# casiacob/ip-parallel-optimal-control

Hardware: AMD Instinct MI355X
Metric: KKT Newton-steps/sec at (horizon N x batch) (higher is better)
Workload: dtype f64; 1 GPU; cartpole nx=4 nu=1 N=200 global batch=4096 (BASELINE c3), 4096 per GPU; layout=tiled, horizon=200, batch_per_gpu=4096, global_batch=4096, lanes_per_trajectory=32, parallelism=trajectory-sharded x1

## Files before the change

### include/noc_hip.h

```cpp
#ifndef NOC_HIP_H
#define NOC_HIP_H

#ifdef __cplusplus
extern "C" {
#endif

#define NOC_ABI_VERSION 5

int noc_abi_version(void);
const char* noc_build_hash(void);
const char* noc_last_error(void);
int noc_kkt_supported(int nx, int nu);
int noc_kkt_default_lanes(int nx, int nu, int N);
int noc_kkt_pick_lanes(int nx, int nu, int N, int B);
int noc_kkt_gains_on_chip(int nx, int nu, int N, int lanes);
void noc_debug_set_ablation(int bits);

int noc_kkt_solve(int nx, int nu, int N, int B, int lanes,
                  const double* A, const double* Bm, const double* Q, const double* R,
                  const double* M, const double* r, const double* q, const double* c,
                  const double* P, const double* p, const double* x0, const double* reg,
                  const int* active,
                  double* dx, double* du, double* pred, int* feasible,
                  double* K, double* d, double* S, double* v, void* stream);
// ... 53 lines not shown
  int Bt, N;
  int lanes;
  int flags;
  double *x, *u, *x0;
  double *A, *B, *Q, *R, *M, *r, *P;
  double *cx, *cu, *lc, *lam;
  double *dx, *du, *pred, *K, *d;
  int *feasible;
  int *phase, *kkt_active, *it, *inner, *total_it, *kkt_solves;
  int *repeats;
  const int *order;
  double *bp, *rp, *rinc, *cost, *hu, *gnorm, *reg;
} noc_ipm_ws;

int noc_family_supported(const noc_family* fam);
int noc_ipm_init(const noc_ipm_ws* ws, double bp0, void* stream);
int noc_ipm_prepare(const noc_family* fam, const noc_ipm_ws* ws, int mode, int terminal,
                    void* stream);
int noc_ipm_trial(const noc_family* fam, const noc_ipm_ws* ws, int mode, void* stream);
int noc_ipm_step(const noc_family* fam, const noc_ipm_ws* ws, int mode, int terminal, int lanes,
                 void* stream);
int noc_ipm_rollout(const noc_family* fam, const noc_ipm_ws* ws, void* stream);
int noc_ipm_step_main(const noc_family* fam, const noc_ipm_ws* ws, int mode, int terminal,
                      void* stream);
int noc_ipm_promote(const noc_ipm_ws* ws, void* stream);

#define NOC_FIELD_A 0
#define NOC_FIELD_B 1
#define NOC_FIELD_Q 2
#define NOC_FIELD_R 3
#define NOC_FIELD_M 4
int noc_kkt_compact_supported(const noc_family* fam, int N, int lanes);
int noc_compact_width(const noc_family* fam, int field);
int noc_kkt_solve_compact(const noc_family* fam, int N, int B, int lanes,
                          const double* A, const double* Bm, const double* Q, const double* R,
                          const double* M, const double* r, const double* P, const double* x0,
                          const double* reg, const int* active,
                          double* dx, double* du, double* pred, int* feasible,
                          double* K, double* d, double* S, double* v, void* stream);
int noc_blocks_expand(const noc_family* fam, int N, int B, int lanes,
                      const double* cA, const double* cB, const double* cQ, const double* cR,
                      const double* cM, double* A, double* Bm, double* Q, double* R, double* M,
                      void* stream);
int noc_ipm_prepare_compact(const noc_family* fam, const noc_ipm_ws* ws, int mode, int terminal,
                            void* stream);
int noc_ipm_step_compact(const noc_family* fam, const noc_ipm_ws* ws, int mode, int terminal,
                         int lanes, void* stream);
int noc_ipm_step_main_compact(const noc_family* fam, const noc_ipm_ws* ws, int mode, int terminal,
                              void* stream);

int noc_ipm_solve_supported(const noc_family* fam, int N, int lanes);
int noc_debug_phase_cycles(long long* out, int n, int reset);
int noc_debug_traj_times(long long* out, int n);
int noc_ipm_solve(const noc_family* fam, const noc_ipm_ws* ws, int mode, int terminal, double bp0,
                  int max_solves, void* stream);

#define NOC_TRAJ_PARAM_DOUBLES 32
#define NOC_TP_GOAL 0
#define NOC_TP_WX 8
#define NOC_TP_WU 16
#define NOC_TP_WF 20
#define NOC_TP_UBOUND 28
int noc_traj_params_supported(const noc_family* fam, int N, int lanes);
int noc_ipm_solve_params(const noc_family* fam, const noc_ipm_ws* ws, const double* params,
                         int mode, int terminal, double bp0, int max_solves, void* stream);
int noc_ipm_prepare_params(const noc_family* fam, const noc_ipm_ws* ws, const double* params,
// ... 65 lines not shown
```

### ip-parallel-optimal-control_amd/csrc/block_struct.h

```cpp
#pragma once
#include <hip/hip_runtime.h>

#include <cstdint>
#include <utility>

#include "ipm_family.h"

namespace noc {

template <class F, int... I>
NOC_DEV void static_for_seq(F&& f, std::integer_sequence<int, I...>) {
  (f(std::integral_constant<int, I>{}), ...);
}
template <int N, class F>
NOC_DEV void static_for(F&& f) {
  static_for_seq(f, std::make_integer_sequence<int, N>{});
}

enum BlockKind : int {
  BK_VAR = 0,
  BK_ZERO,
  BK_ONE,
  BK_DT,
  BK_EXPR_A,
  BK_EXPR_B,
  BK_LIT,
  BK_PA,
  BK_PB,
  BK_WX
};

template <int N>
struct KindTable {
  int kind[N] = {};
  int pos[N] = {};
  int idx[N] = {};
  double lit[N] = {};
  double delta[N] = {};
  int nv = 0;
};

template <int KIND, int NX, int NU>
struct GenPattern {
  static constexpr int NZ = NX + NU;
  static constexpr bool kLinear = KIND == NOC_FAMILY_LINEAR;
  static constexpr bool kDiscrete = Fam<KIND, NX, NU>::kDiscrete;
  static constexpr bool kGenCost = Fam<KIND, NX, NU>::kGenCost;
  static constexpr bool jvar(int k) {
    if constexpr (KIND == NOC_FAMILY_PENDULUM) return gen::pendulum_jac_var[k] != 0;
    else if constexpr (KIND == NOC_FAMILY_CARTPOLE) return gen::cartpole_jac_var[k] != 0;
// ... 114 lines not shown
  for (int i = 0; i < NU; ++i)
    for (int j = i; j < NU; ++j) {
      const int e = Sym<NU>::idx(i, j);
      const bool h = G::hnz((NX + i) * G::NZ + NX + j) || G::hnz((NX + j) * G::NZ + NX + i);
      const int ci = NX * NX + i * NU + j, cj = NX * NX + j * NU + i;
      if (!ON || h || i == j) kt_set(t, e, BK_VAR);
      else if (G::kGenCost) {
        if (G::cvar(ci) || G::cvar(cj)) kt_set(t, e, BK_VAR);
        else kt_set(t, e, BK_LIT, 0.5 * (G::cconst(ci) + G::cconst(cj)));
      } else {
        kt_set(t, e, BK_ZERO);
      }
    }
  return t;
}
template <int KIND, int NX, int NU, bool ON>
constexpr KindTable<NX * NU> table_M() {
  using G = GenPattern<KIND, NX, NU>;
  KindTable<NX * NU> t{};
  for (int i = 0; i < NX; ++i)
    for (int j = 0; j < NU; ++j) {
      const int e = i * NU + j, ck = NX * NX + NU * NU + e;
      if (!ON || G::hnz(i * G::NZ + NX + j)) kt_set(t, e, BK_VAR);
      else if (G::kGenCost) {
        if (G::cvar(ck)) kt_set(t, e, BK_VAR);
        else kt_set(t, e, BK_LIT, G::cconst(ck));
      } else {
        kt_set(t, e, BK_ZERO);
      }
    }
  return t;
}

template <int N>
constexpr uint64_t nz_mask(const KindTable<N>& t) {
  uint64_t m = 0;
  for (int e = 0; e < N; ++e)
    if (t.kind[e] != BK_ZERO) m |= (uint64_t)1 << e;
  return m;
}

template <int KIND, int NX, int NU, bool ON>
struct BlockStruct {
  static_assert(NX * NX <= 64, "structure masks hold up to 64 entries");
  static constexpr bool kOn = ON;
  template <int F>
  static constexpr auto table() {
    if constexpr (F == BF_A) return table_A<KIND, NX, NU, ON>();
    else if constexpr (F == BF_B) return table_B<KIND, NX, NU, ON>();
    else if constexpr (F == BF_Q) return table_Q<KIND, NX, NU, ON>();
    else if constexpr (F == BF_R) return table_R<KIND, NX, NU, ON>();
    else return table_M<KIND, NX, NU, ON>();
  }
  template <int F>
  static constexpr int size() {
    if constexpr (F == BF_A) return NX * NX;
    else if constexpr (F == BF_B || F == BF_M) return NX * NU;
    else if constexpr (F == BF_Q) return Sym<NX>::SZ;
    else return Sym<NU>::SZ;
  }
  template <int F>
  static constexpr int nv() { return table<F>().nv; }
  static constexpr uint64_t kNzA = nz_mask(table_A<KIND, NX, NU, ON>());
  static constexpr uint64_t kNzB = nz_mask(table_B<KIND, NX, NU, ON>());
  static constexpr bool nzA(int k, int j) { return ((kNzA >> (k * NX + j)) & 1) != 0; }
  static constexpr bool nzB(int k, int j) { return ((kNzB >> (k * NU + j)) & 1) != 0; }
// ... 58 lines not shown
```

### ip-parallel-optimal-control_amd/csrc/kkt_compact.hip

```cpp
#include <hip/hip_runtime.h>

#include "../../include/noc_hip.h"
#include "block_struct.h"
#include "noc_internal.h"
#include "small_linalg.h"

namespace noc {

#ifndef NOC_CUSTOM_FAMILY
template <int KIND, int NX, int NU, int L>
hipError_t launch_kkt_compact(const noc_family& prm, const KKTArgs& a, hipStream_t stream);

#define NOC_COMPACT_FAMILIES(X) X(NOC_FAMILY_CARTPOLE, 4, 1) X(NOC_FAMILY_PENDULUM, 2, 1)

template <int KIND, int NX, int NU>
__global__ __launch_bounds__(256) void blocks_expand_kernel(noc_family prm, ExpandArgs e) {
  using BS = BlockStruct<KIND, NX, NU, true>;
  const long long t = (long long)blockIdx.x * blockDim.x + threadIdx.x;
  const int L = e.lanes;
  const Chunks ch(e.N, L);
  if (t >= (long long)e.B * ch.cmax * L) return;
  const int b = (int)(t / ((long long)ch.cmax * L));
  const int rem = (int)(t % ((long long)ch.cmax * L));
  const int j = rem / L, l = rem % L;
// ... 25 lines not shown
    default: return -1;
  }
}

template <int KIND, int NX, int NU>
static hipError_t dispatch_t(const noc_family& p, const KKTArgs& a, int lanes, hipStream_t stream) {
  switch (lanes) {
    case 64: return launch_kkt_compact<KIND, NX, NU, 64>(p, a, stream);
    case 32: return launch_kkt_compact<KIND, NX, NU, 32>(p, a, stream);
    case 16: return launch_kkt_compact<KIND, NX, NU, 16>(p, a, stream);
    case 8: return launch_kkt_compact<KIND, NX, NU, 8>(p, a, stream);
    default: return hipErrorInvalidValue;
  }
}

static bool compact_family(const noc_family& p) {
#define X(K, NX, NU) if (p.kind == K && p.nx == NX && p.nu == NU) return true;
  NOC_COMPACT_FAMILIES(X)
#undef X
  return false;
}

bool kkt_compact_supported(const noc_family& p, int lanes) {
  return compact_family(p) && (lanes == 8 || lanes == 16 || lanes == 32 || lanes == 64);
}

int compact_width(const noc_family& p, int field) {
#define X(K, NX, NU) if (p.kind == K && p.nx == NX && p.nu == NU) return width_t<K, NX, NU>(field);
  NOC_COMPACT_FAMILIES(X)
#undef X
  return -1;
}

hipError_t kkt_compact_dispatch(const noc_family& p, const KKTArgs& a, int lanes, hipStream_t stream) {
#define X(K, NX, NU) if (p.kind == K && p.nx == NX && p.nu == NU) return dispatch_t<K, NX, NU>(p, a, lanes, stream);
  NOC_COMPACT_FAMILIES(X)
#undef X
  return hipErrorInvalidValue;
}

hipError_t blocks_expand(const noc_family& p, const ExpandArgs& e, hipStream_t stream) {
  const long long cmax = (e.N + e.lanes - 1) / e.lanes;
  const unsigned grid = (unsigned)(((long long)e.B * cmax * e.lanes + 255) / 256);
#define X(K, NX, NU)                                                                              \
  if (p.kind == K && p.nx == NX && p.nu == NU) {                                                  \
    hipLaunchKernelGGL((blocks_expand_kernel<K, NX, NU>), dim3(grid), dim3(256), 0, stream, p, e); \
    return hipGetLastError();                                                                     \
  }
  NOC_COMPACT_FAMILIES(X)
#undef X
  return hipErrorInvalidValue;
}

#else

bool kkt_compact_supported(const noc_family&, int) { return false; }
int compact_width(const noc_family&, int) { return -1; }
hipError_t kkt_compact_dispatch(const noc_family&, const KKTArgs&, int, hipStream_t) { return hipErrorInvalidValue; }
hipError_t blocks_expand(const noc_family&, const ExpandArgs&, hipStream_t) { return hipErrorInvalidValue; }

#endif

}
```

### ip-parallel-optimal-control_amd/csrc/kkt_compact_src.h

```cpp
#pragma once
#include <hip/hip_runtime.h>

#include "block_struct.h"
#include "kkt_scan_impl.h"

namespace noc {

template <class BS, int NX, int NU, int L>
struct CompactSrc {
  using Struct = BS;
  const KKTArgs& a;
  const noc_family& p;
  int traj, l, cmax;
  size_t tN;
  template <int F, bool LAST = false>
  NOC_DEV void field(const double* base, int j, double* full) const {
    constexpr int EV = BS::template nv<F>();
    double v[EV > 0 ? EV : 1];
    if constexpr (EV > 0) tload_pol<EV, L, LAST>(base, traj, j, l, cmax, v);
    BS::template expand<F>(p, v, full);
  }
  template <int PART, bool LAST = false>
  NOC_DEV void stage_part(int s, int j, double reg, StageData<NX, NU>& st) const {
    constexpr bool REST = PART != 2, WQ = PART != 1, WAB = REST && PART != 3;
    (void)s;
    (void)reg;
    if constexpr (WAB) {
      field<BF_A>(a.A, j, st.A.v);
      field<BF_B>(a.Bm, j, st.B.v);
    }
    if constexpr (WQ) field<BF_Q, LAST>(a.Q, j, st.Q.v);
    if constexpr (REST) {
      field<BF_R, LAST>(a.R, j, st.R.v);
      field<BF_M, LAST>(a.M, j, st.M.v);
      tload_pol<NU, L, LAST>(a.r, traj, j, l, cmax, st.r.v);
    }
  }
  NOC_DEV void stage(int s, int j, double reg, StageData<NX, NU>& st) const { stage_part<0>(s, j, reg, st); }
  NOC_DEV void stage_last(int s, int j, double reg, StageData<NX, NU>& st) const {
    stage_part<0, true>(s, j, reg, st);
  }
  NOC_DEV void ab(int s, int j, Mat<NX, NX>& A, Mat<NX, NU>& Bm, Vec<NX>& c) const {
    (void)s;
    field<BF_A, true>(a.A, j, A.v);
    field<BF_B, true>(a.Bm, j, Bm.v);
    set_zero(c);
  }
  NOC_DEV void cvec(int, int, Vec<NX>& c) const { set_zero(c); }
};

template <int KIND, int NX, int NU, int L, int CACHE, bool BIG>
__global__ __launch_bounds__(256, BIG ? 1 : NOC_KKT_WAVES_PER_SIMD) void kkt_scan_compact_kernel(noc_family prm,
                                                                                             KKTArgs a) {
  static_assert(L <= 64, "one-wave segments");
  const int tid = blockIdx.x * blockDim.x + threadIdx.x;
  if constexpr (BIG) asm volatile("" ::: "a255");
  const int traj = tid / L;
  const bool dead = traj >= a.B || (a.active && a.active[traj] == 0);
  const bool wave_live = __any(!dead);
  if (dead) {
    if (!wave_live && a.lds_out && a.mode != MODE_BWD && !(a.ablate & 6)) __syncthreads();
    return;
  }
  using BS = BlockStruct<KIND, NX, NU, true>;
  const int l = tid % L;
  const int cmax = a.N / L + (a.N % L ? 1 : 0);
  const CompactSrc<BS, NX, NU, L> src{a, prm, traj, l, cmax, (size_t)traj * a.N};
  kkt_scan_wave_src<NX, NU, L, false, true, CompactSrc<BS, NX, NU, L>, CACHE, true, BIG, false, false, false,
                    true>(a, traj, l, src);
}

template <int KIND, int NX, int NU, int L>
hipError_t launch_kkt_compact(const noc_family& prm, const KKTArgs& a_in, hipStream_t stream) {
  KKTArgs a = a_in;
  const long long threads = (long long)a.B * L;
  constexpr int CC = kkt_cache_len<NX, NU, L>();
  const int cmax = a.N / L + (a.N % L ? 1 : 0);
  const bool cached = CC > 0 && cmax <= CC && !(a.ablate & 8);
  constexpr bool kHasBig = (L == 64 || L == 32) && NX >= 3 && NX <= 4;
  const bool big = kHasBig && (threads + 63) / 64 <= kkt_device_simds() && kkt_big_enabled();
  const size_t slots1 = (a.mode == MODE_BWD || (!a.dx && !a.du)) ? 0 : kkt_lds_bytes_rt(NX, NU, a.N, L);
  const int wpb = kkt_waves_per_block((threads + 63) / 64, slots1);
  const size_t lds = slots1 * wpb;
  a.lds_out = slots1 > 0 ? 1 : 0;
  a.ab_slots = 0;
  a.lds_base = 0;
  a.tiled = 1;
  const int block = 64 * wpb;
  const unsigned grid = (unsigned)((threads + block - 1) / block);
  if (!a.lds_out && (!a.K || !a.d)) return hipErrorInvalidValue;
  if (cached) {
    if constexpr (CC > 0)
      hipLaunchKernelGGL((kkt_scan_compact_kernel<KIND, NX, NU, L, CC, false>), dim3(grid), dim3(block), lds, stream,
                         prm, a);
  } else if (big) {
    if constexpr (kHasBig)
      hipLaunchKernelGGL((kkt_scan_compact_kernel<KIND, NX, NU, L, 0, true>), dim3(grid), dim3(block), lds, stream,
                         prm, a);
  } else {
    hipLaunchKernelGGL((kkt_scan_compact_kernel<KIND, NX, NU, L, 0, false>), dim3(grid), dim3(block), lds, stream,
                       prm, a);
  }
  return hipGetLastError();
}

}
```

### ip-parallel-optimal-control_amd/csrc/kkt_scan_impl.h

```cpp
#pragma once
#include <hip/hip_runtime.h>

#include <type_traits>

#include "small_linalg.h"
#include "noc_internal.h"

#pragma clang fp contract(fast)

#ifndef NOC_KKT_WAVES_PER_SIMD
#define NOC_KKT_WAVES_PER_SIMD 2
#endif


namespace noc {

#ifdef NOC_SCAN_STAMPS
constexpr int kStampWaves = 65536, kStampSlots = 8;
__device__ long long g_scan_stamps[kStampWaves][kStampSlots][2];
#define NOC_STAMP(i)                                                                         \
  do {                                                                                       \
    const unsigned wv_ = (blockIdx.x * blockDim.x + threadIdx.x) >> 6;                      \
    if ((threadIdx.x & 63) == 0 && wv_ < kStampWaves) {                                      \
      g_scan_stamps[wv_][i][0] = (long long)__builtin_amdgcn_s_memrealtime();                \
// ... 449 lines not shown
    NOC_UNROLL for (int k = 0; k < NX; ++k) s += Y[k][i] * w[k];
    e1.nu[i] = s;
  }
  set_zero(e1.A);
  set_zero(e1.b);
  set_zero(e1.C);
}

template <int NX, int NU, int L, bool AFF, bool TILED>
struct ArgsSrc {
  using Struct = DenseBlocks<NX, NU>;
  const KKTArgs& a;
  int traj, l, cmax;
  size_t tN;
  NOC_DEV void stage(int s, int j, double reg, StageData<NX, NU>& st) const {
    load_stage<NX, NU, L, AFF, TILED>(a, traj, tN + s, j, l, cmax, reg, st);
  }
  template <int PART, bool LAST = false>
  NOC_DEV void stage_part(int s, int j, double reg, StageData<NX, NU>& st) const {
    load_stage<NX, NU, L, AFF, TILED, PART, LAST>(a, traj, tN + s, j, l, cmax, reg, st);
  }
  NOC_DEV void stage_last(int s, int j, double reg, StageData<NX, NU>& st) const {
    load_stage<NX, NU, L, AFF, TILED, 0, true>(a, traj, tN + s, j, l, cmax, reg, st);
  }
  NOC_DEV void ab(int s, int j, Mat<NX, NX>& A, Mat<NX, NU>& Bm, Vec<NX>& c) const {
    load_AB<NX, NU, L, AFF, TILED>(a, traj, tN + s, j, l, cmax, A, Bm, c);
  }
  NOC_DEV void cvec(int s, int j, Vec<NX>& c) const {
    if constexpr (TILED) tload<NX, L>(a.c, traj, j, l, cmax, c.v);
    else gload<NX>(a.c + (tN + s) * NX, c.v);
  }
};

template <int NX, int NU, int L, bool AFF, bool TILED, class SRC, int CACHE = 0, bool HANDOFF = true,
          bool BIG = false, bool NT3 = false, bool AB = (BIG && ab_supported<NX, NU>()), bool IO0 = false,
          bool PEEL = false>
NOC_DEV void kkt_scan_wave_src(const KKTArgs& a, const int traj, const int l, const SRC& src) {
  constexpr int KD = kd_width<NX, NU>();
  using ST = typename SRC::Struct;
  if (traj >= a.B) return;
  if (a.active && a.active[traj] == 0) return;
  const int N = a.N;
  const int base = N / L, rem = N % L;
  const int len = base + (l < rem ? 1 : 0);
  const int start = l * base + (l < rem ? l : rem);
  const bool last = (l == L - 1);
  const int io = IO0 ? 0 : traj;
  const double reg = a.reg ? a.reg[io] : 0.0;
  const size_t tN = (size_t)traj * N;
  const int cmax = base + (rem ? 1 : 0);
  constexpr int LW = L > 64 ? 64 : L;
  constexpr int W = L / LW;
  static_assert(W == 1 || W == 2, "segments of up to two waves");
  const int wv = l / LW, lw = l % LW;
  double* join = nullptr;
  if constexpr (W > 1) join = lds_join<NX, NU>(N, a.lds_out != 0);
  (void)wv;
  (void)lw;
  (void)join;
  lds_double* lab = nullptr;
  int abn = 0;
  if constexpr (AB) {
    abn = (CACHE == 0 && a.mode != MODE_FWD && !(a.ablate & (16 | 64))) ? a.ab_slots : 0;
    if (abn > 0) lab = lds_ab<NX, NU>(a.lds_base, a.ab_slots);
  }
  NOC_STAMP_DECL;
  NOC_STAMP(0);
  StageData<NX, NU> cache[CACHE > 0 ? CACHE : 1];
  if constexpr (CACHE > 0) {
    if (a.mode != MODE_FWD) {
      NOC_UNROLL for (int jj = 0; jj < CACHE; ++jj)
        if (jj < len) src.stage(start + jj, jj, reg, cache[jj]);
    }
  }

  Mat<NX, NX> Phi;
  Vec<NX> phi;
  Mat<NX, NX> hA;
  Mat<NX, NU> hB;
  Vec<NX> hc;
  bool handed = false;
  SRC src_re = src;
  if (a.ablate & 16) { src_re.traj = traj & 1; src_re.tN = (size_t)(traj & 1) * N; }
  if (a.mode != MODE_FWD) {
    Elem<NX> e;
    set_zero(e.b);
    set_zero(e.C);
    if (last) {
      set_zero(e.A);
      set_zero(e.nu);
      gload_sym<NX, true>(a.P + (size_t)traj * NX * NX, e.J);
      if constexpr (AFF) { if (a.p) gload<NX>(a.p + (size_t)traj * NX, e.nu.v); }
    } else {
      set_identity(e.A);
      set_zero(e.nu);
      set_zero(e.J);
    }
    if constexpr (CACHE > 0) {
      NOC_UNROLL for (int jj = CACHE - 1; jj >= 0; --jj)
        if (jj < len) prepend<NX, NU, AFF, ST>(e, cache[jj], reg);
    } else {
      for (int s = start + len - 1; s >= start; --s) {
        StageData<NX, NU> st;
        src.stage(s, s - start, reg, st);
        if constexpr (AB) { if (s - start < abn) ab_store<NX, NU>(lab, s - start, st.A, st.B); }
        prepend<NX, NU, AFF, ST>(e, st, reg);
      }
    }
    NOC_STAMP(1); NOC_ISA_MARK("phase", 1);
    if constexpr (W == 1) {
      if (!(a.ablate & 1)) rev_scan_sklansky<NX, L, 0, (NX <= 2 || BIG)>(e);
    } else {
      if (!(a.ablate & 1)) {
        combine_sklansky<NX, false, 0, true>(e);
// ... 149 lines not shown
          NOC_UNROLL for (int j = 0; j < NX; ++j) {
            double u = 0.0;
            NOC_UNROLL for (int k = 0; k < NX; ++k) if (ST::nzF(k, j)) u += Phi(i, k) * F(k, j);
            Pn(i, j) = u;
          }
        }
        Phi = Pn;
      }
    };
    const int sfirst = start + len - 1;
    constexpr std::true_type kFirst{};
    constexpr std::false_type kLater{};
    if constexpr (CACHE > 0) {
      NOC_UNROLL for (int jj = CACHE - 1; jj >= 0; --jj)
        if (jj < len) riccati_stage(start + jj, cache[jj], jj == len - 1);
    } else {
      bool split = false;
      if constexpr (AB) split = abn > 0;
      if (split) {
        if constexpr (AB) {
          const int jl = len < abn ? len : abn;
          for (int s = start + len - 1; s >= start + jl; --s) {
            StageData<NX, NU> st;
            stage3(s, st);
            riccati_stage(s, st, s == sfirst);
          }
          for (int s = start + jl - 1; s >= start; --s) {
            StageData<NX, NU> st;
            src_re.template stage_part<3, NT3>(s, s - start, reg, st);
            ab_load<NX, NU>(lab, s - start, st.A, st.B);
            riccati_stage(s, st, s == sfirst);
          }
        }
      } else if constexpr (HANDOFF) {
        int s = sfirst;
        if (PEEL && len > 1) {
          StageData<NX, NU> st;
          stage3(s, st);
          riccati_stage(s, st, kFirst);
          --s;
        }
        for (; s > start; --s) {
          StageData<NX, NU> st;
          stage3(s, st);
          riccati_stage(s, st, kLater);
        }
        if (len > 0) {
          StageData<NX, NU> st;
          stage3(start, st);
          riccati_stage(start, st, len == 1);
          hA = st.A;
          hB = st.B;
          if constexpr (AFF) hc = st.c; else set_zero(hc);
          handed = a.mode == MODE_FULL && !(a.ablate & 32);
        }
      } else {
        for (int s = start + len - 1; s >= start; --s) {
          StageData<NX, NU> st;
          stage3(s, st);
          riccati_stage(s, st, s == sfirst);
        }
      }
    }
    segment_sum_and<LW>(pred, feas, (int)__lane_id());
    if constexpr (W > 1) {
      constexpr int PO = Sym<NX>::SZ + 2 * NX;
// ... 31 lines not shown
          NOC_UNROLL for (int u = 0; u < NU; ++u) if (ST::nzB(i, u)) t += Bm(i, u) * Kk[u * NX + j];
          F(i, j) = t;
        }
        double t = cc[i];
        NOC_UNROLL for (int u = 0; u < NU; ++u) if (ST::nzB(i, u)) t += Bm(i, u) * Kk[NU * NX + u];
        f[i] = t;
      }
      Mat<NX, NX> Pn;
      NOC_UNROLL for (int i = 0; i < NX; ++i) {
        double t = phi[i];
        NOC_UNROLL for (int k = 0; k < NX; ++k) if (AFF || ST::nzf(k)) t += Phi(i, k) * f[k];
        phi[i] = t;
        NOC_UNROLL for (int j = 0; j < NX; ++j) {
          double u = 0.0;
          NOC_UNROLL for (int k = 0; k < NX; ++k) if (ST::nzF(k, j)) u += Phi(i, k) * F(k, j);
          Pn(i, j) = u;
        }
      }
      Phi = Pn;
    }
  }

  Vec<NX> x0;
  set_zero(x0);
  if (a.x0) gload<NX>(a.x0 + (size_t)traj * NX, x0.v);
  if (l == 0) {
    NOC_UNROLL for (int i = 0; i < NX; ++i) {
      double t = phi[i];
      NOC_UNROLL for (int k = 0; k < NX; ++k) t += Phi(i, k) * x0[k];
      phi[i] = t;
    }
    set_zero(Phi);
  }
  affine_prefix_sklansky<NX, LW>(Phi, phi);
  Vec<NX> x;
  wave_shift_up1<NX>(phi.v, x.v);
  if (l == 0) x = x0;
  if constexpr (W > 1) {
    constexpr int XO = Sym<NX>::SZ + NX;
    if (wv == 0 && lw == LW - 1) NOC_UNROLL for (int i = 0; i < NX; ++i) join[XO + i] = phi[i];
    Mat<NX, NX> oP;
    if (wv == 1) wave_shift_up1<NX * NX>(Phi.v, oP.v);
    __syncthreads();
    if (wv == 1) {
      Vec<NX> xw;
      NOC_UNROLL for (int i = 0; i < NX; ++i) xw[i] = join[XO + i];
      if (lw == 0) {
        x = xw;
      } else {
        NOC_UNROLL for (int i = 0; i < NX; ++i) {
          double t = x[i];
          NOC_UNROLL for (int k = 0; k < NX; ++k) t += oP(i, k) * xw[k];
          x[i] = t;
        }
      }
    }
  }
  NOC_STAMP(4); NOC_ISA_MARK("phase", 4);
  double* slot = lds_slots<NX, NU, L>(N);
  const bool via_lds = a.lds_out != 0;
  const bool kd_lds = via_lds && a.mode == MODE_FULL;
  Mat<NX, NX> nA;
  Mat<NX, NU> nB;
  double nK[NU * (NX + 1)];
  Vec<NX> nc;
  auto fetch = [&](int s) {
// ... 40 lines not shown
            NOC_UNROLL for (int i = 0; i < NU * (NX + 1); ++i) Kk[i] = slot[s * KD + i];
          } else {
            load_Kd<NX, NU, L, TILED>(a, traj, tN + s, jj, l, cmax, Kk);
          }
          Vec<NX> cc;
          if constexpr (AFF) cc = cache[jj].c; else set_zero(cc);
          fwd_stage(s, cache[jj].A, cache[jj].B, cc, Kk);
        }
      }
    }
  } else {
    int s0 = start;
    if constexpr (AB) {
      if (abn > 0) {
        const int jl = len < abn ? len : abn;
        for (int s = start; s < start + jl; ++s) {
          Mat<NX, NX> A;
          Mat<NX, NU> Bm;
          Vec<NX> cc;
          ab_load<NX, NU>(lab, s - start, A, Bm);
          set_zero(cc);
          if constexpr (AFF) { if (a.c) src_re.cvec(s, s - start, cc); }
          double Kk[NU * (NX + 1)];
          if (kd_lds) {
            NOC_UNROLL for (int i = 0; i < NU * (NX + 1); ++i) Kk[i] = slot[s * KD + i];
          } else {
            load_Kd<NX, NU, L, TILED>(a, traj, tN + s, s - start, l, cmax, Kk);
          }
          fwd_stage(s, A, Bm, cc, Kk);
        }
        s0 = start + jl;
      }
    }
    if (s0 < start + len) {
      if (handed && s0 == start) {
        nA = hA;
        nB = hB;
        nc = hc;
        if (kd_lds) {
          NOC_UNROLL for (int i = 0; i < NU * (NX + 1); ++i) nK[i] = slot[start * KD + i];
        } else {
          load_Kd<NX, NU, L, TILED>(a, traj, tN + start, 0, l, cmax, nK);
        }
      } else {
        fetch(s0);
      }
    }
    for (int s = s0; s < start + len; ++s) {
      const Mat<NX, NX> A = nA;
      const Mat<NX, NU> Bm = nB;
      const Vec<NX> cc = nc;
      double Kk[NU * (NX + 1)];
      NOC_UNROLL for (int i = 0; i < NU * (NX + 1); ++i) Kk[i] = nK[i];
      if (s + 1 < start + len) fetch(s + 1);
      fwd_stage(s, A, Bm, cc, Kk);
    }
  }
  NOC_STAMP(5); NOC_ISA_MARK("phase", 5);
  if (!via_lds) {
    if (last && a.dx) gstore<NX>(a.dx + (tN + traj + N) * NX, x.v);
    return;
  }
  if (last) NOC_UNROLL for (int i = 0; i < NX; ++i) slot[N * KD + i] = x[i];
  __syncthreads();
  if (a.dx) {
    double* dst = a.dx + (tN + traj) * NX;
    if constexpr (NX % 2 == 0) {
      constexpr int H = NX / 2;
      double2* dst2 = reinterpret_cast<double2*>(dst);
      for (int i = l; i < (N + 1) * H; i += L) {
        const int s = i / H, e = 2 * (i - s * H);
        noc_dbl2 v;
        v.x = slot[s * KD + e];
        v.y = slot[s * KD + e + 1];
        __builtin_nontemporal_store(v, reinterpret_cast<noc_dbl2*>(dst2 + i));
      }
    } else {
      for (int i = l; i < (N + 1) * NX; i += L) {
        const int s = i / NX;
        dst[i] = slot[s * KD + (i - s * NX)];
      }
    }
  }
  if (a.du) {
    double* dst = a.du + tN * NU;
    for (int i = l; i < N * NU; i += L) {
      const int s = i / NU;
      dst[i] = slot[s * KD + NX + (i - s * NU)];
    }
  }
  NOC_STAMP(6);
}

template <int NX, int NU, int L, bool AFF, bool TILED, int CACHE = 0, bool HANDOFF = true,
          bool BIG = false, bool NT3 = false>
NOC_DEV void kkt_scan_wave(const KKTArgs& a, const int traj, const int l) {
  const int cmax = a.N / L + (a.N % L ? 1 : 0);
  const ArgsSrc<NX, NU, L, AFF, TILED> src{a, traj, l, cmax, (size_t)traj * a.N};
  kkt_scan_wave_src<NX, NU, L, AFF, TILED, ArgsSrc<NX, NU, L, AFF, TILED>, CACHE, HANDOFF, BIG, NT3,
                    (BIG && ab_supported<NX, NU>()), false, true>(a, traj, l, src);
}

template <int NX, int NU, int L, bool AFF, bool TILED, int CACHE, bool BIG = false, bool NT3 = false>
__global__ __launch_bounds__(L > 64 ? L : 256, (L > 64 || BIG) ? 1 : NOC_KKT_WAVES_PER_SIMD) void kkt_scan_kernel(KKTArgs a) {
  const int tid = blockIdx.x * blockDim.x + threadIdx.x;
  if constexpr (L > 64 || BIG) asm volatile("" ::: "a255");
  const int traj = tid / L;
  if constexpr (L <= 64) {
    const bool dead = traj >= a.B || (a.active && a.active[traj] == 0);
    const bool wave_live = __any(!dead);
    if (dead) {
      if (!wave_live && a.lds_out && a.mode != MODE_BWD && !(a.ablate & 6)) __syncthreads();
      return;
    }
  }
  kkt_scan_wave<NX, NU, L, AFF, TILED, CACHE, true, BIG, NT3 && TILED && CACHE == 0>(a, traj, tid % L);
}

template <int NX, int NU, int L>
constexpr int kkt_cache_len() { return (NX <= 2 && L >= 32) ? 2 : 0; }


template <int NX, int NU, int L, bool AFF>
hipError_t launch_kkt(const KKTArgs& a_in, hipStream_t stream) {
// ... 90 lines not shown
```

### ip-parallel-optimal-control_amd/csrc/noc_abi.hip

```cpp
#include <hip/hip_runtime.h>

#include <cstdint>
#include <cstdio>
#include <string>

#include "../../include/noc_hip.h"
#include "noc_internal.h"
#include "small_linalg.h"

namespace noc {
static std::string kkt_shapes_str();
}

namespace {
thread_local std::string g_last_error;
int g_ablate = 0;

int fail(int code, const std::string& msg) {
  g_last_error = msg;
  return code;
}

int check_ptr(const void* p, const char* name, bool required, unsigned align = 16) {
  if (!p) return required ? fail(-2, std::string("required pointer is NULL: ") + name) : 0;
// ... 144 lines not shown
                    "kkt_scan launch");
}

int noc_kkt_solve(int nx, int nu, int N, int B, int lanes, const double* A, const double* Bm,
                  const double* Q, const double* R, const double* M, const double* r,
                  const double* q, const double* c, const double* P, const double* p,
                  const double* x0, const double* reg, const int* active, double* dx, double* du,
                  double* pred, int* feasible, double* K, double* d, double* S, double* v,
                  void* stream) {
  return kkt_common(noc::MODE_FULL, 0, nx, nu, N, B, lanes, A, Bm, Q, R, M, r, q, c, P, p, x0, reg,
                    active, dx, du, pred, feasible, K, d, S, v, stream);
}

int noc_kkt_solve_tiled(int nx, int nu, int N, int B, int lanes, const double* A,
                        const double* Bm, const double* Q, const double* R, const double* M,
                        const double* r, const double* q, const double* c, const double* P,
                        const double* p, const double* x0, const double* reg, const int* active,
                        double* dx, double* du, double* pred, int* feasible, double* K, double* d,
                        double* S, double* v, void* stream) {
  return kkt_common(noc::MODE_FULL, 1, nx, nu, N, B, lanes, A, Bm, Q, R, M, r, q, c, P, p, x0,
                    reg, active, dx, du, pred, feasible, K, d, S, v, stream);
}

int noc_kkt_compact_supported(const noc_family* fam, int N, int lanes) {
  return (fam && N >= 1 && noc::kkt_compact_supported(*fam, lanes)) ? 1 : 0;
}

int noc_compact_width(const noc_family* fam, int field) {
  if (!fam) return fail(-1, "family is NULL");
  const int w = noc::compact_width(*fam, field);
  return w < 0 ? fail(-1, "noc_compact_width: unsupported family or field") : w;
}

static int check_compact_dims(const noc_family* fam, int N, int B, int lanes) {
  if (!fam) return fail(-1, "family is NULL");
  if (N < 1) return fail(-1, "horizon N must be >= 1");
  if (B < 0) return fail(-1, "batch B must be >= 0");
  if (!noc::kkt_compact_supported(*fam, lanes))
    return fail(-1, "compact blocks: unsupported family or lanes (" + std::to_string(lanes) +
                        "); pendulum and cart-pole at lanes 8, 16, 32 or 64 (noc_kkt_compact_supported)");
  return 0;
}

int noc_kkt_solve_compact(const noc_family* fam, int N, int B, int lanes, const double* A,
                          const double* Bm, const double* Q, const double* R, const double* M,
                          const double* r, const double* P, const double* x0, const double* reg,
                          const int* active, double* dx, double* du, double* pred, int* feasible,
                          double* K, double* d, double* S, double* v, void* stream) {
  if (check_compact_dims(fam, N, B, lanes)) return -1;
  const void* req[] = {A, Bm, Q, R, M, r, P};
  const char* names[] = {"A", "B", "Q", "R", "M", "r", "P"};
  for (int i = 0; i < 7; ++i)
    if (check_ptr(req[i], names[i], true)) return -1;
  if (check_ptr(x0, "x0", false) || check_ptr(K, "K", false) || check_ptr(d, "d", false) ||
      check_ptr(S, "S", false) || check_ptr(v, "v", false) || check_ptr(dx, "dx", false) ||
      check_ptr(du, "du", false) || check_ptr(reg, "reg", false, 8) ||
      check_ptr(pred, "pred", false, 8) || check_ptr(feasible, "feasible", false, 4) ||
      check_ptr(active, "active", false, 4))
    return -1;
  if (B == 0) return 0;
  const int nx = fam->nx, nu = fam->nu;
  const bool on_chip = (dx || du) && noc::kkt_lds_bytes_rt(nx, nu, N, lanes) > 0;
  if ((!K || !d) && !on_chip) {
    fail(-2, "K and d are required (workspace) unless noc_kkt_gains_on_chip() is 1");
    return -1;
  }
// ... 595 lines not shown
```

### ip-parallel-optimal-control_amd/csrc/noc_internal.h

```cpp
#pragma once
#include <hip/hip_runtime.h>

#include <cstdlib>

#include "../../include/noc_hip.h"

#ifndef NOC_FAMILIES_DEF
#define NOC_FAMILIES_DEF "families.def"
#endif
#ifndef NOC_KKT_SHAPES_DEF
#define NOC_KKT_SHAPES_DEF "kkt_shapes.def"
#endif

#if defined(__HIP_DEVICE_COMPILE__) && !defined(__gfx950__)
#error "libnoc_hip targets gfx950 (MI355X) only: LDS budgets and cache policies are sized for it"
#endif

namespace noc {

enum KKTMode : int { MODE_FULL = 0, MODE_BWD = 1, MODE_FWD = 2 };

struct KKTArgs {
  int N, B, mode;
  int ab_slots;
// ... 101 lines not shown
    }                                                                                           \
  } while (0)
int wide_set_decision_trace(const DecisionTrace& t);
int debug_set_decision_trace(double* buf, int cap, int ntraj);

struct DerivArgs {
  int N, B;
  const double *x, *u, *bp;
  double *cx, *cu, *cxx, *cuu, *cxu, *fx, *fu, *fxx, *fuu, *fxu;
};
struct LqrArgs {
  int nx, nu, N, B;
  const double *lam, *cu, *cxx, *cuu, *cxu, *fu, *fxx, *fuu, *fxu;
  double *ru, *Q, *R, *M;
};
hipError_t derivatives(const noc_family& p, const DerivArgs& a, hipStream_t s);
hipError_t final_cost_derivs(const noc_family& p, int B, const double* xN, double* grad,
                             double* hess, hipStream_t s);
hipError_t costates(int nx, int N, int B, const double* lamT, const double* cx, const double* fx,
                    double* lam, int sequential, hipStream_t s);
hipError_t lqr_params(const LqrArgs& a, hipStream_t s);
hipError_t traj_feasibility(const noc_family& p, int N, int B, const double* x, const double* u,
                            int* ok, hipStream_t s);
hipError_t total_cost(const noc_family& p, int N, int B, const double* x, const double* u,
                      const double* bp, double* cost, hipStream_t s);

hipError_t kkt_dispatch(int nx, int nu, const KKTArgs& a, int lanes, hipStream_t stream);
hipError_t kkt_group_dispatch(int nx, int nu, const KKTArgs& a, hipStream_t stream);
template <int NX, int NU>
hipError_t kkt_dispatch_shape(const KKTArgs& a, int lanes, hipStream_t stream);
bool kkt_supported(int nx, int nu);
bool kkt_compact_supported(const noc_family& p, int lanes);
int compact_width(const noc_family& p, int field);
hipError_t kkt_compact_dispatch(const noc_family& p, const KKTArgs& a, int lanes, hipStream_t stream);
struct ExpandArgs {
  int N, B, lanes;
  const double *cA, *cB, *cQ, *cR, *cM;
  double *A, *Bm, *Q, *R, *M;
};
hipError_t blocks_expand(const noc_family& p, const ExpandArgs& e, hipStream_t stream);
int kkt_default_lanes(int nx, int nu, int N);
int kkt_pick_lanes(int nx, int nu, int N, int B);

hipError_t ipm_prepare(const noc_family& p, const noc_ipm_ws& w, int mode, int terminal,
                       bool compact, hipStream_t s);
hipError_t ipm_trial(const noc_family& p, const noc_ipm_ws& w, int mode, hipStream_t s);
hipError_t ipm_rollout(const noc_family& p, const noc_ipm_ws& w, hipStream_t s);
hipError_t ipm_prepare_main(const noc_family& p, const noc_ipm_ws& w, int mode, int terminal,
                            bool compact, hipStream_t s);
hipError_t ipm_promote(const noc_ipm_ws& w, hipStream_t s);
hipError_t ipm_init(const noc_ipm_ws& w, double bp0, hipStream_t s);
bool ipm_solve_supported(const noc_family& p, int N, int lanes);
bool ddp_supported(const noc_family& p);
long long ddp_record_doubles(int nx, int nu);
hipError_t ddp_solve(const noc_family& p, int N, int Bt, const double* x0, double* u,
                     double* work, int* iterations, int* passes, int* done, double bp0,
                     int max_passes, int flags, hipStream_t s);
struct DdpBwdArgs {
  int N, B;
  const double *Vx, *Vxx, *reg_param;
  const double *cx, *cu, *cxx, *cuu, *cxu, *fx, *fu, *fxx, *fuu, *fxu;
  double *k, *K, *pred, *Hu;
  int* feasible;
};
hipError_t ddp_bwd_pass(int nx, int nu, const DdpBwdArgs& a, hipStream_t s);
hipError_t nonlin_rollout(const noc_family& p, int N, int B, const double* K, const double* k,
// ... 37 lines not shown
```

### ip-parallel-optimal-control_amd/csrc/small_linalg.h

```cpp
#pragma once
#include <hip/hip_runtime.h>

namespace noc {

#define NOC_DEV __device__ __forceinline__
#define NOC_UNROLL _Pragma("unroll")

#ifdef NOC_ISA_MARKS
#define NOC_ISA_MARK(tag, k) asm volatile("; NOC_MARK " tag " %0" ::"i"(k))
#else
#define NOC_ISA_MARK(tag, k) do { } while (0)
#endif

template <int R, int C>
struct Mat {
  double v[R * C];
  NOC_DEV double& operator()(int i, int j) { return v[i * C + j]; }
  NOC_DEV double operator()(int i, int j) const { return v[i * C + j]; }
};

template <int N>
struct Vec {
  double v[N];
  NOC_DEV double& operator[](int i) { return v[i]; }
  NOC_DEV double operator[](int i) const { return v[i]; }
};

template <int N>
struct Sym {
  static constexpr int SZ = N * (N + 1) / 2;
  double v[SZ];
  static __host__ __device__ constexpr int idx(int i, int j) {
    return i <= j ? i * N - (i * (i - 1)) / 2 + (j - i) : j * N - (j * (j - 1)) / 2 + (i - j);
  }
  NOC_DEV double& operator()(int i, int j) { return v[idx(i, j)]; }
  NOC_DEV double operator()(int i, int j) const { return v[idx(i, j)]; }
};

template <int R, int C>
NOC_DEV void set_zero(Mat<R, C>& m) { NOC_UNROLL for (int i = 0; i < R * C; ++i) m.v[i] = 0.0; }
template <int N>
NOC_DEV void set_zero(Vec<N>& m) { NOC_UNROLL for (int i = 0; i < N; ++i) m.v[i] = 0.0; }
template <int N>
NOC_DEV void set_zero(Sym<N>& m) { NOC_UNROLL for (int i = 0; i < Sym<N>::SZ; ++i) m.v[i] = 0.0; }
template <int N>
// ... 431 lines not shown
```

### ip-parallel-optimal-control_amd/noc/_lib.py

```python
from __future__ import annotations

import ctypes
import os
from typing import Optional

_HERE = os.path.dirname(os.path.abspath(__file__))
LIB_PATH = os.environ.get("NOC_HIP_LIB", os.path.join(_HERE, "_lib", "libnoc_hip.so"))

_COMMON_SOURCES = ("csrc/small_linalg.h", "csrc/noc_internal.h", "csrc/kkt_shapes.def", "Makefile",
                   "../include/noc_hip.h")
KKT_KERNEL_SOURCES = {
    "kkt_scan": ("csrc/kkt_scan_impl.h", "csrc/kkt_scan_2x1.hip", "csrc/kkt_scan_4x1.hip",
                 "csrc/kkt_scan_4x1_l32.hip", "csrc/kkt_scan_4x1_l32nt.hip",
                 "csrc/kkt_scan_4x1_l128.hip", "csrc/kkt_scan_8x4.hip", "csrc/kkt_scan_8x4_l32.hip",
                 "csrc/kkt_scan_8x4_l16.hip", "csrc/kkt_scan_8x4_l8.hip",
                 "csrc/kkt_compact_src.h", "csrc/block_struct.h", "csrc/kkt_compact.hip",
                 "csrc/kkt_scan_compact_pendulum.hip", "csrc/kkt_scan_compact_cartpole_l8.hip",
                 "csrc/kkt_scan_compact_cartpole_l16.hip", "csrc/kkt_scan_compact_cartpole_l32.hip",
                 "csrc/kkt_scan_compact_cartpole_l64.hip") + _COMMON_SOURCES,
    "kkt_group8": ("csrc/kkt_group_impl.h", "csrc/kkt_group8_impl.h", "csrc/kkt_group.hip")
    + _COMMON_SOURCES,
}

ABI_VERSION = 5
# ... 37 lines not shown
                    "dx", "du", "pred", "K", "d"]
WS_ONE_STAGE = 1
WS_RESUME = 2
WS_NO_REPEAT_SKIP = 4
WS_INT_FIELDS = ["feasible", "phase", "kkt_active", "it", "inner", "total_it", "kkt_solves",
                 "repeats"]
WS_STATE_FIELDS = ["bp", "rp", "rinc", "cost", "hu", "gnorm", "reg"]


FIELD_A, FIELD_B, FIELD_Q, FIELD_R, FIELD_M = range(5)
WS_OPT_FIELDS = ["order"]


class NocIpmWs(ctypes.Structure):
    _fields_ = ([("Bt", _i), ("N", _i), ("lanes", _i), ("flags", _i)]
                + [(f, _dp) for f in WS_DOUBLE_FIELDS]
                + [(f, _dp) for f in WS_INT_FIELDS] + [(f, _dp) for f in WS_OPT_FIELDS]
                + [(f, _dp) for f in WS_STATE_FIELDS])


_fp = ctypes.POINTER(NocFamily)
_wp = ctypes.POINTER(NocIpmWs)
SIGNATURES.update({
    "noc_family_supported": (_i, [_fp]),
    "noc_ipm_init": (_i, [_wp, ctypes.c_double, _dp]),
    "noc_ipm_prepare": (_i, [_fp, _wp, _i, _i, _dp]),
    "noc_ipm_trial": (_i, [_fp, _wp, _i, _dp]),
    "noc_ipm_step": (_i, [_fp, _wp, _i, _i, _i, _dp]),
    "noc_ipm_rollout": (_i, [_fp, _wp, _dp]),
    "noc_ipm_step_main": (_i, [_fp, _wp, _i, _i, _dp]),
    "noc_ipm_promote": (_i, [_wp, _dp]),
    "noc_kkt_compact_supported": (_i, [_fp, _i, _i]),
    "noc_compact_width": (_i, [_fp, _i]),
    "noc_kkt_solve_compact": (_i, [_fp, _i, _i, _i] + [_dp] * 10 + [_dp] * 8 + [_dp]),
    "noc_blocks_expand": (_i, [_fp, _i, _i, _i] + [_dp] * 10 + [_dp]),
    "noc_ipm_prepare_compact": (_i, [_fp, _wp, _i, _i, _dp]),
    "noc_ipm_step_compact": (_i, [_fp, _wp, _i, _i, _i, _dp]),
    "noc_ipm_step_main_compact": (_i, [_fp, _wp, _i, _i, _dp]),
    "noc_ipm_solve_supported": (_i, [_fp, _i, _i]),
    "noc_debug_phase_cycles": (_i, [ctypes.POINTER(ctypes.c_longlong), _i, _i]),
    "noc_debug_traj_times": (_i, [ctypes.POINTER(ctypes.c_longlong), _i]),
    "noc_ipm_solve": (_i, [_fp, _wp, _i, _i, ctypes.c_double, _i, _dp]),
    "noc_traj_params_supported": (_i, [_fp, _i, _i]),
    "noc_ipm_solve_params": (_i, [_fp, _wp, _dp, _i, _i, ctypes.c_double, _i, _dp]),
    "noc_ipm_prepare_params": (_i, [_fp, _wp, _dp, _i, _i, _dp]),
    "noc_ipm_trial_params": (_i, [_fp, _wp, _dp, _i, _dp]),
    "noc_ipm_step_params": (_i, [_fp, _wp, _dp, _i, _i, _i, _dp]),
    "noc_derivatives": (_i, [_fp, _i, _i] + [_dp] * 13 + [_dp]),
    "noc_final_cost_derivs": (_i, [_fp, _i, _dp, _dp, _dp, _dp]),
    "noc_costates": (_i, [_i, _i, _i, _dp, _dp, _dp, _dp, _i, _dp]),
    "noc_lqr_params": (_i, [_i] * 4 + [_dp] * 13 + [_dp]),
    "noc_check_feasibility": (_i, [_fp, _i, _i, _dp, _dp, _dp, _dp]),
    "noc_total_cost": (_i, [_fp, _i, _i, _dp, _dp, _dp, _dp, _dp]),
    "noc_ddp_work_doubles": (ctypes.c_longlong, [_i, _i, _i, _i]),
    "noc_ddp_supported": (_i, [_fp]),
    "noc_ddp_solve": (_i, [_fp, _i, _i] + [_dp] * 6 + [ctypes.c_double, _i, _dp]),
    "noc_ddp_solve_ex": (_i, [_fp, _i, _i] + [_dp] * 6 + [ctypes.c_double, _i, _i, _dp]),
    "noc_ddp_bwd_pass": (_i, [_i] * 4 + [_dp] * 18 + [_dp]),
    "noc_nonlin_rollout": (_i, [_fp, _i, _i] + [_dp] * 6 + [_dp]),
    "noc_ddp_params_supported": (_i, [_fp]),
    "noc_ddp_solve_params": (_i, [_fp, _i, _i] + [_dp] * 6 + [_dp, ctypes.c_double, _i, _i, _dp]),
    "noc_derivatives_params": (_i, [_fp, _i, _i] + [_dp] * 13 + [_dp, _dp]),
    "noc_final_cost_derivs_params": (_i, [_fp, _i, _dp, _dp, _dp, _dp, _dp]),
    "noc_check_feasibility_params": (_i, [_fp, _i, _i, _dp, _dp, _dp, _dp, _dp]),
    "noc_total_cost_params": (_i, [_fp, _i, _i, _dp, _dp, _dp, _dp, _dp, _dp]),
})
# ... 115 lines not shown
```

Before: 83.95 million trajectory-KKT-steps/s.

## Keep compressed A/B records in registers from backward pass for forward sweep

In the compact cartpole/pendulum scan kernel, the backward Riccati sweep now packs the compressed A and B blocks of the first KEEP stages of each lane's chunk into a small register buffer. The forward sweep then reuses these records instead of reloading them from global memory, and prefetches the next stage's dynamics before the affine prefix scan. The aim is to cut global-memory reads and load latency in the forward pass. The cost is extra register pressure from the keep buffer (7 records for cartpole), which could lower occupancy or cause spills.

```diff
diff --git a/include/noc_hip.h b/include/noc_hip.h
--- a/include/noc_hip.h
+++ b/include/noc_hip.h
@@ -109,6 +109,7 @@
 #define NOC_FIELD_M 4
 int noc_kkt_compact_supported(const noc_family* fam, int N, int lanes);
 int noc_compact_width(const noc_family* fam, int field);
+int noc_kkt_compact_keep(const noc_family* fam, int lanes);
 int noc_kkt_solve_compact(const noc_family* fam, int N, int B, int lanes,
                           const double* A, const double* Bm, const double* Q, const double* R,
                           const double* M, const double* r, const double* P, const double* x0,
diff --git a/ip-parallel-optimal-control_amd/csrc/block_struct.h b/ip-parallel-optimal-control_amd/csrc/block_struct.h
--- a/ip-parallel-optimal-control_amd/csrc/block_struct.h
+++ b/ip-parallel-optimal-control_amd/csrc/block_struct.h
@@ -7,15 +7,6 @@
 #include "ipm_family.h"
 
 namespace noc {
-
-template <class F, int... I>
-NOC_DEV void static_for_seq(F&& f, std::integer_sequence<int, I...>) {
-  (f(std::integral_constant<int, I>{}), ...);
-}
-template <int N, class F>
-NOC_DEV void static_for(F&& f) {
-  static_for_seq(f, std::make_integer_sequence<int, N>{});
-}
 
 enum BlockKind : int {
   BK_VAR = 0,
@@ -196,6 +187,11 @@
   return t;
 }
 
+constexpr int compact_keep(int kind, int lanes) {
+  (void)lanes;
+  return kind == NOC_FAMILY_CARTPOLE ? 7 : 4;
+}
+
 template <int N>
 constexpr uint64_t nz_mask(const KindTable<N>& t) {
   uint64_t m = 0;
diff --git a/ip-parallel-optimal-control_amd/csrc/kkt_compact.hip b/ip-parallel-optimal-control_amd/csrc/kkt_compact.hip
--- a/ip-parallel-optimal-control_amd/csrc/kkt_compact.hip
+++ b/ip-parallel-optimal-control_amd/csrc/kkt_compact.hip
@@ -81,6 +81,10 @@
   return -1;
 }
 
+int kkt_compact_keep(const noc_family& p, int lanes) {
+  return kkt_compact_supported(p, lanes) ? compact_keep(p.kind, lanes) : -1;
+}
+
 hipError_t kkt_compact_dispatch(const noc_family& p, const KKTArgs& a, int lanes, hipStream_t stream) {
 #define X(K, NX, NU) if (p.kind == K && p.nx == NX && p.nu == NU) return dispatch_t<K, NX, NU>(p, a, lanes, stream);
   NOC_COMPACT_FAMILIES(X)
@@ -105,6 +109,7 @@
 
 bool kkt_compact_supported(const noc_family&, int) { return false; }
 int compact_width(const noc_family&, int) { return -1; }
+int kkt_compact_keep(const noc_family&, int) { return -1; }
 hipError_t kkt_compact_dispatch(const noc_family&, const KKTArgs&, int, hipStream_t) { return hipErrorInvalidValue; }
 hipError_t blocks_expand(const noc_family&, const ExpandArgs&, hipStream_t) { return hipErrorInvalidValue; }
 
diff --git a/ip-parallel-optimal-control_amd/csrc/kkt_compact_src.h b/ip-parallel-optimal-control_amd/csrc/kkt_compact_src.h
--- a/ip-parallel-optimal-control_amd/csrc/kkt_compact_src.h
+++ b/ip-parallel-optimal-control_amd/csrc/kkt_compact_src.h
@@ -47,9 +47,20 @@
     set_zero(c);
   }
   NOC_DEV void cvec(int, int, Vec<NX>& c) const { set_zero(c); }
+  static constexpr int kNvA = BS::template nv<BF_A>(), kNvB = BS::template nv<BF_B>();
+  static constexpr int kRecAB = kNvA + kNvB;
+  NOC_DEV void pack_ab(const Mat<NX, NX>& A, const Mat<NX, NU>& Bm, double* rec) const {
+    BS::template compress<BF_A>(A.v, rec);
+    BS::template compress<BF_B>(Bm.v, rec + kNvA);
+  }
+  NOC_DEV void unpack_ab(const double* rec, Mat<NX, NX>& A, Mat<NX, NU>& Bm, Vec<NX>& c) const {
+    BS::template expand<BF_A>(p, rec, A.v);
+    BS::template expand<BF_B>(p, rec + kNvA, Bm.v);
+    set_zero(c);
+  }
 };
 
-template <int KIND, int NX, int NU, int L, int CACHE, bool BIG>
+template <int KIND, int NX, int NU, int L, int CACHE, bool BIG, int KEEP = 0>
 __global__ __launch_bounds__(256, BIG ? 1 : NOC_KKT_WAVES_PER_SIMD) void kkt_scan_compact_kernel(noc_family prm,
                                                                                              KKTArgs a) {
   static_assert(L <= 64, "one-wave segments");
@@ -67,7 +78,7 @@
   const int cmax = a.N / L + (a.N % L ? 1 : 0);
   const CompactSrc<BS, NX, NU, L> src{a, prm, traj, l, cmax, (size_t)traj * a.N};
   kkt_scan_wave_src<NX, NU, L, false, true, CompactSrc<BS, NX, NU, L>, CACHE, true, BIG, false, false, false,
-                    true>(a, traj, l, src);
+                    true, KEEP>(a, traj, l, src);
 }
 
 template <int KIND, int NX, int NU, int L>
@@ -78,6 +89,7 @@
   const int cmax = a.N / L + (a.N % L ? 1 : 0);
   const bool cached = CC > 0 && cmax <= CC && !(a.ablate & 8);
   constexpr bool kHasBig = (L == 64 || L == 32) && NX >= 3 && NX <= 4;
+  constexpr int KP = compact_keep(KIND, L);
   const bool big = kHasBig && (threads + 63) / 64 <= kkt_device_simds() && kkt_big_enabled();
   const size_t slots1 = (a.mode == MODE_BWD || (!a.dx && !a.du)) ? 0 : kkt_lds_bytes_rt(NX, NU, a.N, L);
   const int wpb = kkt_waves_per_block((threads + 63) / 64, slots1);
@@ -95,10 +107,10 @@
                          prm, a);
   } else if (big) {
     if constexpr (kHasBig)
-      hipLaunchKernelGGL((kkt_scan_compact_kernel<KIND, NX, NU, L, 0, true>), dim3(grid), dim3(block), lds, stream,
+      hipLaunchKernelGGL((kkt_scan_compact_kernel<KIND, NX, NU, L, 0, true, KP>), dim3(grid), dim3(block), lds, stream,
                          prm, a);
   } else {
-    hipLaunchKernelGGL((kkt_scan_compact_kernel<KIND, NX, NU, L, 0, false>), dim3(grid), dim3(block), lds, stream,
+    hipLaunchKernelGGL((kkt_scan_compact_kernel<KIND, NX, NU, L, 0, false, KP>), dim3(grid), dim3(block), lds, stream,
                        prm, a);
   }
   return hipGetLastError();
diff --git a/ip-parallel-optimal-control_amd/csrc/kkt_scan_impl.h b/ip-parallel-optimal-control_amd/csrc/kkt_scan_impl.h
--- a/ip-parallel-optimal-control_amd/csrc/kkt_scan_impl.h
+++ b/ip-parallel-optimal-control_amd/csrc/kkt_scan_impl.h
@@ -505,12 +505,21 @@
   }
 };
 
+template <class SRC, int KEEP>
+constexpr int keep_rec_doubles() {
+  if constexpr (KEEP > 0) return SRC::kRecAB > 0 ? SRC::kRecAB : 1;
+  else return 1;
+}
+
 template <int NX, int NU, int L, bool AFF, bool TILED, class SRC, int CACHE = 0, bool HANDOFF = true,
           bool BIG = false, bool NT3 = false, bool AB = (BIG && ab_supported<NX, NU>()), bool IO0 = false,
-          bool PEEL = false>
+          bool PEEL = false, int KEEP = 0>
 NOC_DEV void kkt_scan_wave_src(const KKTArgs& a, const int traj, const int l, const SRC& src) {
   constexpr int KD = kd_width<NX, NU>();
   using ST = typename SRC::Struct;
+  static_assert(KEEP == 0 || (PEEL && HANDOFF && CACHE == 0 && !AB && !AFF && L <= 64),
+                "KEEP: the streamed, non-affine one-wave hand-off path with the peeled first stage");
+  constexpr int REC = keep_rec_doubles<SRC, KEEP>();
   if (traj >= a.B) return;
   if (a.active && a.active[traj] == 0) return;
   const int N = a.N;
@@ -553,6 +562,16 @@
   Mat<NX, NU> hB;
   Vec<NX> hc;
   bool handed = false;
+  double kbuf[KEEP > 0 ? KEEP : 1][REC];
+  (void)kbuf;
+#define NOC_KEEP_PUT(J, STAGE)                                                        \
+  do {                                                                                \
+    double rec_[REC];                                                                 \
+    src.pack_ab((STAGE).A, (STAGE).B, rec_);                                          \
+    NOC_UNROLL for (int k_ = 0; k_ < KEEP; ++k_) {                                    \
+      if ((J) == k_) { NOC_UNROLL for (int i_ = 0; i_ < REC; ++i_) kbuf[k_][i_] = rec_[i_]; } \
+    }                                                                                 \
+  } while (0)
   SRC src_re = src;
   if (a.ablate & 16) { src_re.traj = traj & 1; src_re.tN = (size_t)(traj & 1) * N; }
   if (a.mode != MODE_FWD) {
@@ -768,6 +787,27 @@
             riccati_stage(s, st, s == sfirst);
           }
         }
+      } else if constexpr (KEEP > 0) {
+        if (len > 1) {
+          StageData<NX, NU> st;
+          stage3(sfirst, st);
+          riccati_stage(sfirst, st, kFirst);
+          NOC_KEEP_PUT(len - 1, st);
+        }
+        for (int jj = cmax - 2; jj >= 1; --jj) {
+          if (jj <= len - 2) {
+            StageData<NX, NU> st;
+            stage3(start + jj, st);
+            riccati_stage(start + jj, st, kLater);
+            NOC_KEEP_PUT(jj, st);
+          }
+        }
+        if (len > 0) {
+          StageData<NX, NU> st;
+          stage3(start, st);
+          riccati_stage(start, st, len == 1);
+          NOC_KEEP_PUT(0, st);
+        }
       } else if constexpr (HANDOFF) {
         int s = sfirst;
         if (PEEL && len > 1) {
@@ -865,6 +905,18 @@
     }
     set_zero(Phi);
   }
+  Mat<NX, NX> pA;
+  Mat<NX, NU> pB;
+  Vec<NX> pc;
+  const int kept = (KEEP > 0 && a.mode == MODE_FULL && !(a.ablate & 32)) ? KEEP : 0;
+  bool pre = false;
+  if constexpr (KEEP > 0) {
+    if (len > kept) {
+      src_re.ab(start + kept, kept, pA, pB, pc);
+      pre = true;
+    }
+  }
+  (void)kept;
   affine_prefix_sklansky<NX, LW>(Phi, phi);
   Vec<NX> x;
   wave_shift_up1<NX>(phi.v, x.v);
@@ -971,8 +1023,41 @@
         s0 = start + jl;
       }
     }
+    if constexpr (KEEP > 0) {
+      if (kept > 0) {
+        static_for<KEEP>([&](auto KC) {
+          constexpr int k = decltype(KC)::value;
+          if (k < len) {
+            const int s = start + k;
+            Mat<NX, NX> A;
+            Mat<NX, NU> Bm;
+            Vec<NX> cc;
+            double rec[REC];
+            static_for<REC>([&](auto IC) { rec[decltype(IC)::value] = kbuf[k][decltype(IC)::value]; });
+            src.unpack_ab(rec, A, Bm, cc);
+            double Kk[NU * (NX + 1)];
+            if (kd_lds) {
+              NOC_UNROLL for (int i = 0; i < NU * (NX + 1); ++i) Kk[i] = slot[s * KD + i];
+            } else {
+              load_Kd<NX, NU, L, TILED>(a, traj, tN + s, k, l, cmax, Kk);
+            }
+            fwd_stage(s, A, Bm, cc, Kk);
+          }
+        });
+        s0 = start + (len < KEEP ? len : KEEP);
+      }
+    }
     if (s0 < start + len) {
-      if (handed && s0 == start) {
+      if (pre) {
+        nA = pA;
+        nB = pB;
+        nc = pc;
+        if (kd_lds) {
+          NOC_UNROLL for (int i = 0; i < NU * (NX + 1); ++i) nK[i] = slot[s0 * KD + i];
+        } else {
+          load_Kd<NX, NU, L, TILED>(a, traj, tN + s0, s0 - start, l, cmax, nK);
+        }
+      } else if (handed && s0 == start) {
         nA = hA;
         nB = hB;
         nc = hc;
@@ -1029,6 +1114,7 @@
     }
   }
   NOC_STAMP(6);
+#undef NOC_KEEP_PUT
 }
 
 template <int NX, int NU, int L, bool AFF, bool TILED, int CACHE = 0, bool HANDOFF = true,
diff --git a/ip-parallel-optimal-control_amd/csrc/noc_abi.hip b/ip-parallel-optimal-control_amd/csrc/noc_abi.hip
--- a/ip-parallel-optimal-control_amd/csrc/noc_abi.hip
+++ b/ip-parallel-optimal-control_amd/csrc/noc_abi.hip
@@ -200,6 +200,11 @@
   return w < 0 ? fail(-1, "noc_compact_width: unsupported family or field") : w;
 }
 
+int noc_kkt_compact_keep(const noc_family* fam, int lanes) {
+  if (!fam) return fail(-1, "family is NULL");
+  return noc::kkt_compact_keep(*fam, lanes);
+}
+
 static int check_compact_dims(const noc_family* fam, int N, int B, int lanes) {
   if (!fam) return fail(-1, "family is NULL");
   if (N < 1) return fail(-1, "horizon N must be >= 1");
diff --git a/ip-parallel-optimal-control_amd/csrc/noc_internal.h b/ip-parallel-optimal-control_amd/csrc/noc_internal.h
--- a/ip-parallel-optimal-control_amd/csrc/noc_internal.h
+++ b/ip-parallel-optimal-control_amd/csrc/noc_internal.h
@@ -157,6 +157,7 @@
 bool kkt_supported(int nx, int nu);
 bool kkt_compact_supported(const noc_family& p, int lanes);
 int compact_width(const noc_family& p, int field);
+int kkt_compact_keep(const noc_family& p, int lanes);
 hipError_t kkt_compact_dispatch(const noc_family& p, const KKTArgs& a, int lanes, hipStream_t stream);
 struct ExpandArgs {
   int N, B, lanes;
diff --git a/ip-parallel-optimal-control_amd/csrc/small_linalg.h b/ip-parallel-optimal-control_amd/csrc/small_linalg.h
--- a/ip-parallel-optimal-control_amd/csrc/small_linalg.h
+++ b/ip-parallel-optimal-control_amd/csrc/small_linalg.h
@@ -1,5 +1,7 @@
 #pragma once
 #include <hip/hip_runtime.h>
+
+#include <utility>
 
 namespace noc {
 
@@ -11,6 +13,15 @@
 #else
 #define NOC_ISA_MARK(tag, k) do { } while (0)
 #endif
+
+template <class F, int... I>
+NOC_DEV void static_for_seq(F&& f, std::integer_sequence<int, I...>) {
+  (f(std::integral_constant<int, I>{}), ...);
+}
+template <int N, class F>
+NOC_DEV void static_for(F&& f) {
+  static_for_seq(f, std::make_integer_sequence<int, N>{});
+}
 
 template <int R, int C>
 struct Mat {
diff --git a/ip-parallel-optimal-control_amd/noc/_lib.py b/ip-parallel-optimal-control_amd/noc/_lib.py
--- a/ip-parallel-optimal-control_amd/noc/_lib.py
+++ b/ip-parallel-optimal-control_amd/noc/_lib.py
@@ -93,6 +93,7 @@
     "noc_ipm_promote": (_i, [_wp, _dp]),
     "noc_kkt_compact_supported": (_i, [_fp, _i, _i]),
     "noc_compact_width": (_i, [_fp, _i]),
+    "noc_kkt_compact_keep": (_i, [_fp, _i]),
     "noc_kkt_solve_compact": (_i, [_fp, _i, _i, _i] + [_dp] * 10 + [_dp] * 8 + [_dp]),
     "noc_blocks_expand": (_i, [_fp, _i, _i, _i] + [_dp] * 10 + [_dp]),
     "noc_ipm_prepare_compact": (_i, [_fp, _wp, _i, _i, _dp]),
```

New measurement: 87.29 million trajectory-KKT-steps/s, median of 6. 4.0% higher.
